# AroneyS/galah

Measured on AMD Instinct MI355X. Metric: precluster genome-pairs/sec at 10k genomes (s=1000) + sketch Gbases/s, higher is better.
Workload: dtype u64; 1 GPU; C3: 10000 synthetic genomes x 3000000 bp, clusters of 10, sub rate U(0,0.07), k=21, s=1000, min_ani=0.95; genomes=10000, genome_len=3000000, sketch_size=1000, k=21, parallelism=dp1, mode=lib

## Files before the change

### galah_amd/csrc/api.cpp

```cpp
#include <hip/hip_runtime.h>

#include <algorithm>
#include <chrono>
#include <cmath>
#include <cstdio>
#include <cstdlib>
#include <cstring>
#include <map>
#include <mutex>
#include <new>
#include <string>
#include <thread>
#include <vector>

#include "context.hpp"


namespace gg {

thread_local std::string g_thread_err;

void set_thread_error(const std::string& msg) { g_thread_err = msg; }

gg_status fail(gg_ctx* c, gg_status st, const std::string& msg) {
  if (c) c->err = msg;
  set_thread_error(msg);
  return st;
}

gg_status hip_fail(gg_ctx* c, hipError_t e, const char* what) {
  return fail(c, e == hipErrorOutOfMemory ? GG_ERR_OUT_OF_MEMORY : GG_ERR_HIP,
              std::string(what) + ": " + hipGetErrorString(e));
}

hipError_t scratch(gg_ctx* c, const char* key, size_t bytes, void** out) {
  auto& e = c->scratch[key];
  if (e.second < bytes) {
// ... 733 lines not shown
  a.overflow = b.flags + 2;
  {
    const char* e = getenv("GALAHGPU_INDEX_COST");
    const double k = !weigh_cost ? 0.0 : e && *e ? atof(e) : 0.0;
    const uint64_t n_new = n - n_old;
    const uint64_t npairs = n_old ? n_new * n_old + n_new * (n_new - 1) / 2 : pairs_in_tiles(n, tb, te);
    const double lim = k * (double)c->s * (double)npairs;
    a.cost = b.cost;
    a.cost_limit = k > 0 && lim < 1.8e19 ? (unsigned long long)lim : ~0ull;
  }
  uint64_t* d_count0;
  GG_HIP(c, scratch_t(c, "idx_count0", 1, &d_count0));
  GG_HIP(c, hipMemcpyAsync(d_count0, d_count, sizeof(uint64_t), hipMemcpyDeviceToDevice, st));
  auto launch_pairs = [&](bool guarded) -> gg_status {
    a.build_flags = guarded ? b.flags : nullptr;
    a.ents16 = b.bucket && index_ents16(n);
    GG_HIP(c, timed_launch(c, GG_KERNEL_PAIRS, work, st, [&] { return launch_index_pairs(a, r1 - r0, st); }));
    return GG_OK;
  };
  uint64_t info[2] = {0, 0};
  uint32_t kept = 0;
  uint32_t flags[4] = {0, 0, 0, 0};
  bool built = false, paired = false;
  if (b.bucket && !b.bloom) {
    const uint32_t nbb = index_bucket_bound(total);
    const char* se = getenv("GALAHGPU_INDEX_SPLIT");
    const bool split = !(se && *se == '0');
    if (split) {
      GG_HIP(c, scratch_t(c, "idx_split_cnt", (size_t)256 * n + 1, &b.split_cnt));
      GG_HIP(c, scratch_t(c, "idx_split_off", (size_t)256 * n + 1, &b.split_off));
      GG_HIP(c, scratch_t(c, "idx_split_hist", (size_t)256 * 16 * 256, &b.split_hist));
    }
    b.sort_tmp_bytes = split ? index_split_tmp_bytes(n) : index_bucket_sort_tmp_bytes(total);
    GG_HIP(c, scratch(c, "idx_sort_tmp", b.sort_tmp_bytes, &b.sort_tmp));
    GG_HIP(c, scratch_t(c, "idx_bstart", split ? (size_t)65537 : (size_t)nbb + 1, &b.bstart));
    GG_HIP(c, timed_launch(c, GG_KERNEL_PAIRS_INDEX, total, st, [&] { return index_fill(b, st); }));
    GG_HIP(c, timed_launch(c, GG_KERNEL_PAIRS_INDEX, 0, st, [&] { return index_build_buckets(b, total, nbb, st); }));
    gg_status ps = launch_pairs(true);
    if (ps != GG_OK) return ps;
    uint64_t* h_if;
    GG_HIP(c, host_scratch_t(c, "idx_info", 5, &h_if));
    GG_HIP(c, hipMemcpyAsync(h_if, b.info, 5 * sizeof(uint64_t), hipMemcpyDeviceToHost, st));
    GG_HIP(c, hipStreamSynchronize(st));
    memcpy(info, h_if, sizeof info);
    memcpy(flags, h_if + 2, sizeof flags);
    built = paired = flags[3] == 0;
    if (built && !flags[0] && h_if[4] > a.cost_limit) {
      *costly = true;
      return GG_OK;
    }
  } else {
    uint32_t nbuckets = 0;
    GG_HIP(c, timed_launch(c, GG_KERNEL_PAIRS_INDEX, total, st, [&] { return index_fill(b, st); }));
    GG_HIP(c, hipMemcpyAsync(info, b.info, sizeof info, hipMemcpyDeviceToHost, st));
    if (b.bloom) GG_HIP(c, hipMemcpyAsync(&kept, b.flags + 1, sizeof kept, hipMemcpyDeviceToHost, st));
    if (b.bucket)
      GG_HIP(c, hipMemcpyAsync(&nbuckets, b.bbase + kIndexCoarse, sizeof nbuckets, hipMemcpyDeviceToHost, st));
    GG_HIP(c, hipStreamSynchronize(st));
    if (b.bucket) {
      b.sort_tmp_bytes = index_bucket_sort_tmp_bytes(kept);
      GG_HIP(c, scratch(c, "idx_sort_tmp", b.sort_tmp_bytes, &b.sort_tmp));
      GG_HIP(c, scratch_t(c, "idx_bstart", (size_t)nbuckets + 1, &b.bstart));
      GG_HIP(c, timed_launch(c, GG_KERNEL_PAIRS_INDEX, 0, st,
                             [&] { return index_build_buckets(b, kept, nbuckets, st); }));
      GG_HIP(c, hipMemcpyAsync(flags, b.flags, sizeof flags, hipMemcpyDeviceToHost, st));
      GG_HIP(c, hipStreamSynchronize(st));
      built = flags[3] == 0;
    }
  }
// ... 23 lines not shown
    }
    a.big_map = h_if[5] > kBigMapRun;
  } else if (!paired && !flags[0]) {
    uint64_t cost[2] = {0, 0};
    GG_HIP(c, hipMemcpyAsync(cost, b.info + 4, sizeof cost, hipMemcpyDeviceToHost, st));
    GG_HIP(c, hipStreamSynchronize(st));
    if (cost[0] > a.cost_limit) {
      *costly = true;
      return GG_OK;
    }
    a.big_map = cost[1] > kBigMapRun;
  }
  if (flags[0]) return GG_OK;
  if (!paired) {
    gg_status ps = launch_pairs(false);
    if (ps != GG_OK) return ps;
    GG_HIP(c, hipMemcpyAsync(&flags[2], b.flags + 2, sizeof(uint32_t), hipMemcpyDeviceToHost, st));
    GG_HIP(c, hipStreamSynchronize(st));
  }
  *used = true;
  if (flags[2]) {
    GG_HIP(c, hipMemcpyAsync(d_count, d_count0, sizeof(uint64_t), hipMemcpyDeviceToDevice, st));
    *used = false;
  }
  return GG_OK;
}

}

gg_status pairs_tables(gg_ctx* c, float min_ani, uint32_t** d_cmin, uint32_t** d_sufmin, hipStream_t st) {
  return ensure_cmin(c, min_ani, d_cmin, d_sufmin, st);
}

gg_status sorted_pairs_device(gg_ctx* c, const gg_pair* d_pairs, uint64_t cnt, uint32_t n, gg_pair** d_sorted,
                              hipStream_t st) {
  uint64_t* d_kv;
  void* d_tmp;
  const size_t tmp_bytes = pair_sort_tmp_bytes(cnt, n);
  GG_HIP(c, scratch_t(c, "pair_sort_kv", 5 * std::max<uint64_t>(cnt, 1), &d_kv));
  GG_HIP(c, scratch(c, "pair_sort_tmp", std::max<size_t>(tmp_bytes, 16), &d_tmp));
  uint32_t* d_idx = (uint32_t*)(d_kv + 2 * cnt);
  *d_sorted = (gg_pair*)(d_kv + 3 * cnt);
  if (cnt == 0) return GG_OK;
  GG_HIP(c, sort_pairs_device(d_pairs, cnt, n, d_kv, d_kv + cnt, d_idx, d_idx + cnt, *d_sorted, d_tmp, tmp_bytes, st));
  return GG_OK;
}
// ... 66 lines not shown
                           hipMemcpyHostToDevice, st));
  if (kern == 1) {
    PairsTableLaunch b;
    b.sketches = d_sk;
    b.lens = d_lens;
    b.n = n;
    b.stride = c->s;
    b.segs = d_segs;
    b.n_segs = (uint32_t)c->seg_host.size();
    b.cmin = d_cmin;
    b.tmax = 2 * c->s;
    b.out = d_out;
    b.out_cap = cap;
    b.count = (unsigned long long*)d_count;
    GG_HIP(c, timed_launch(c, GG_KERNEL_PAIRS, work, st, [&] { return launch_pairs_table(b, st); }));
    return GG_OK;
  }
#endif
  return GG_OK;
}

gg_status pairs_range_to_host(gg_ctx* c, const uint64_t* d_sk, const uint32_t* d_lens, uint32_t n,
                              uint64_t tb, uint64_t te, float min_ani, std::vector<gg_pair>& res,
                              hipStream_t st, uint32_t n_old) {
  if (n < 2 || tb >= te) return GG_OK;
  uint64_t *d_count, *h_count;
  GG_HIP(c, scratch_t(c, "pair_count", 1, &d_count));
  GG_HIP(c, host_scratch_t(c, "pair_count", 1, &h_count));
  uint64_t cap = std::max<uint64_t>(1 << 20, (uint64_t)n * 16);
  const uint64_t all = (uint64_t)n * (n > 0 ? n - 1 : 0) / 2;
  cap = std::min<uint64_t>(cap, std::max<uint64_t>(all, 1));
  for (int attempt = 0; attempt < 2; ++attempt) {
    gg_pair* d_out;
    GG_HIP(c, scratch_t(c, "pair_out", cap, &d_out));
    GG_HIP(c, hipMemsetAsync(d_count, 0, sizeof(uint64_t), st));
    gg_status ps = pairs_core(c, d_sk, d_lens, n, tb, te, min_ani, d_out, cap, d_count, st, n_old);
    if (ps != GG_OK) return ps;
    GG_HIP(c, hipMemcpyAsync(h_count, d_count, sizeof(uint64_t), hipMemcpyDeviceToHost, st));
    GG_HIP(c, hipStreamSynchronize(st));
    const uint64_t cnt = *h_count;
    if (cnt <= cap) {
      const size_t at = res.size();
      res.resize(at + cnt);
      if (cnt < kDeviceSortPairs || cnt >= (1ull << 31)) {
        if (cnt) {
          GG_HIP(c, hipMemcpyAsync(res.data() + at, d_out, cnt * sizeof(gg_pair), hipMemcpyDeviceToHost, st));
          GG_HIP(c, hipStreamSynchronize(st));
          std::sort(res.begin() + at, res.end(), [](const gg_pair& x, const gg_pair& y) {
            return x.i != y.i ? x.i < y.i : x.j < y.j;
          });
        }
        return GG_OK;
      }
      uint64_t* d_kv;
      void* d_tmp;
      const size_t tmp_bytes = pair_sort_tmp_bytes(cnt, n);
      GG_HIP(c, scratch_t(c, "pair_sort_kv", 5 * cnt, &d_kv));
      GG_HIP(c, scratch(c, "pair_sort_tmp", std::max<size_t>(tmp_bytes, 16), &d_tmp));
      uint32_t* d_idx = (uint32_t*)(d_kv + 2 * cnt);
      gg_pair* d_sorted = (gg_pair*)(d_kv + 3 * cnt);
      GG_HIP(c, sort_pairs_device(d_out, cnt, n, d_kv, d_kv + cnt, d_idx, d_idx + cnt, d_sorted, d_tmp, tmp_bytes,
                                  st));
      constexpr uint64_t kPairStage = 1ull << 20;
      gg_pair* h_sorted;
      GG_HIP(c, host_scratch_t(c, "pair_sorted", std::min(cnt, kPairStage), &h_sorted));
      for (uint64_t x = 0; x < cnt; x += kPairStage) {
        const uint64_t m = std::min(kPairStage, cnt - x);
        GG_HIP(c, hipMemcpyAsync(h_sorted, d_sorted + x, m * sizeof(gg_pair), hipMemcpyDeviceToHost, st));
        GG_HIP(c, hipStreamSynchronize(st));
        memcpy(res.data() + at + x, h_sorted, m * sizeof(gg_pair));
      }
      return GG_OK;
    }
    cap = cnt;
  }
  return fail(c, GG_ERR_INTERNAL, "pair output sizing failed");
}

double ani_f64(uint32_t common, uint32_t total, int k) {
  const double jaccard = (double)common / (double)total;
  double d = -1.0 * std::log((2.0 * jaccard) / (1.0 + jaccard)) / (double)k;
  d = rust_max(rust_min(d, 1.0), 0.0);
  return 1.0 - d;
}

std::vector<uint32_t> build_cmin(uint32_t s, int k, float min_ani) {
  const uint32_t tmax = 2 * s;
  const double thr = (double)min_ani;
  std::vector<uint32_t> cmin(tmax + 1, 0xFFFFFFFFu);
  for (uint32_t t = 0; t <= tmax; ++t) {
    const uint32_t cmax = std::min(t, s);
    if (!(ani_f64(cmax, t, k) >= thr)) continue;
    uint32_t lo = 0, hi = cmax;
// ... 514 lines not shown
```

### galah_amd/csrc/context.hpp

```cpp
#pragma once

#include <hip/hip_runtime.h>

#include <condition_variable>
#include <cstdlib>
#include <cstring>
#include <functional>
#include <map>
#include <memory>
#include <mutex>
#include <string>
#include <thread>
#include <vector>

#include "gg_internal.hpp"

class MemberPool {
 public:
  explicit MemberPool(size_t n) {
    for (size_t i = 1; i < n; ++i) th_.emplace_back([this, i] { loop(i); });
  }
  ~MemberPool() {
    {
      std::lock_guard<std::mutex> lk(mu_);
// ... 82 lines not shown
  std::unique_ptr<MemberPool> pool;
  std::vector<hipStream_t> peer_streams;
  uint64_t pair_paths[GG_PATH_COUNT] = {};
  int pairs_path = GG_PAIRS_PATH_DEFAULT;
  uint64_t pairs_paths_taken[3] = {};
  uint64_t index_costly = 0;
  uint64_t fallbacks[GG_FALLBACK_COUNT] = {};
  uint64_t inflate_dev_batches = 0;
  uint64_t gz_member_plans = 0, gz_full_plans = 0;
  uint64_t gz_scratch_bytes = 0;
  uint64_t cluster_calls = 0, cluster_rounds = 0;
  uint64_t precluster_calls = 0, precluster_jumps = 0;
  uint64_t scratch_regrows = 0;
  double scratch_regrow_ms = 0;
  double scratch_hint = 1.0;
  std::vector<uint8_t> peer_direct;
  std::vector<hipEvent_t> rep_start, rep_done;
  std::vector<char> rep_live;
  hipEvent_t rows_ready = nullptr;
  hipStream_t copy_stream = nullptr;
  hipEvent_t copy_done = nullptr;
  int host_threads = 0;
  double phase_ms[GG_PHASE_COUNT] = {0};
};

namespace gg {

inline gg_ctx* primary(gg_ctx* c) { return c && !c->devs.empty() ? c->devs[0] : c; }

gg_status fail(gg_ctx* c, gg_status st, const std::string& msg);
gg_status hip_fail(gg_ctx* c, hipError_t e, const char* what);

#define GG_HIP(ctx, expr)                                        \
  do {                                                           \
    hipError_t _e = (expr);                                      \
    if (_e != hipSuccess) return ::gg::hip_fail((ctx), _e, #expr); \
  } while (0)

hipError_t scratch(gg_ctx* c, const char* key, size_t bytes, void** out);
template <typename T>
hipError_t scratch_t(gg_ctx* c, const char* key, size_t count, T** out) {
  void* p = nullptr;
  hipError_t e = scratch(c, key, count * sizeof(T), &p);
  *out = (T*)p;
  return e;
}
hipError_t pinned(gg_ctx* c, size_t bytes, void** out);
hipError_t host_scratch(gg_ctx* c, const char* key, size_t bytes, void** out);
template <typename T>
hipError_t host_scratch_t(gg_ctx* c, const char* key, size_t count, T** out) {
  void* p = nullptr;
  hipError_t e = host_scratch(c, key, count * sizeof(T), &p);
  *out = static_cast<T*>(p);
  return e;
}

gg_status check_runs(gg_ctx* c, const gg_run* runs, uint64_t n_runs, uint32_t n_genomes, uint64_t n_words);
gg_status sketch_core(gg_ctx* c, const uint32_t* d_words, uint64_t n_words, const gg_run* runs,
                      uint64_t n_runs, uint32_t n_genomes, uint64_t* d_out, uint32_t* d_lens,
                      const uint32_t* d_row_of, hipStream_t st);
gg_status pairs_core(gg_ctx* c, const uint64_t* d_sk, const uint32_t* d_lens, uint32_t n,
                     uint64_t tb, uint64_t te, float min_ani, gg_pair* d_out, uint64_t cap,
                     uint64_t* d_count, hipStream_t st, uint32_t n_old = 0);
constexpr uint64_t kDeviceSortPairs = 4096;
gg_status pairs_range_to_host(gg_ctx* c, const uint64_t* d_sk, const uint32_t* d_lens, uint32_t n,
                              uint64_t tb, uint64_t te, float min_ani, std::vector<gg_pair>& res,
                              hipStream_t st, uint32_t n_old = 0);

gg_status cluster_device(gg_ctx* c, uint32_t n, const gg_pair* d_pairs, const float* d_ani, uint64_t n_pairs, float T,
                         uint32_t* d_rep_of, hipStream_t st);
gg_status preclusters_device(gg_ctx* c, uint32_t n, const gg_pair* d_pairs, uint64_t n_pairs, uint32_t* d_members,
                             uint32_t* d_offsets, uint32_t* n_sets, gg_local_pair* d_local, uint64_t* d_pair_offsets,
                             hipStream_t st);
gg_status ani_f32_device(gg_ctx* c, const gg_pair* d_pairs, uint64_t n_pairs, float* d_ani, double* d_ani_f64,
                         uint64_t* n_rechecked, hipStream_t st);
struct AniFlagged;
using AniProducer = std::function<hipError_t(double E, AniFlagged* list, uint64_t cap, unsigned long long* count)>;
gg_status ani_flagged_passes(gg_ctx* c, const char* who, uint64_t n_items, const AniProducer& produce, float* d_ani,
                             double* d_ani_f64, uint32_t mirror_m, uint64_t* n_flagged, hipStream_t st);
gg_status ani_matrix_device(gg_ctx* c, const uint64_t* d_sk, const uint32_t* d_lens, uint32_t n, const uint32_t* d_rows,
                            uint32_t m, uint32_t* d_common, uint32_t* d_total, float* d_ani, gg_matrix_summary* sum,
                            hipStream_t st);
gg_status ani_matrix_groups_device(gg_ctx* c, const uint64_t* d_sk, const uint32_t* d_lens, uint32_t n,
                                   const uint32_t* d_members, const uint32_t* offsets, uint32_t n_groups,
                                   uint32_t* d_common, uint32_t* d_total, float* d_ani, gg_matrix_summary* sum,
                                   hipStream_t st);
struct MatrixPrep {
  const uint32_t *pos_row, *pos_len, *piece, *piece_cnt;
  uint32_t m;
  uint64_t n_entries, n_columns, column_entries;
// ... 85 lines not shown
```

### galah_amd/csrc/gg_internal.hpp

```cpp
#pragma once

#include <hip/hip_runtime.h>

#include <cstdint>
#include <memory>
#include <string>
#include <vector>

#include "../../include/galahgpu.h"

namespace gg {

constexpr uint64_t kEmpty = ~0ull;

enum SketchStatus : uint32_t {
  kSketchOk = 0,
  kSketchRetryLarger = 1,
  kSketchRetrySmaller = 2,
  kSketchRetrySet = 3,
};

constexpr uint32_t kFlagOverflow = 1u;
constexpr uint32_t kFlagSawMax = 2u;
constexpr uint32_t kFlagSetMode = 4u;
// ... 317 lines not shown
  unsigned long long* count;
  uint32_t max_split_log2;
  uint32_t* overflow;
  const uint32_t* build_flags = nullptr;
  bool ents16 = false;
  const unsigned long long* cost = nullptr;
  unsigned long long cost_limit = ~0ull;
  bool big_map = false;
  bool border = false;
};
hipError_t index_fill(const IndexBuild& b, hipStream_t st);
hipError_t index_build(const IndexBuild& b, uint64_t total, uint32_t sh, uint32_t end_bit, hipStream_t st);
hipError_t index_build_buckets(const IndexBuild& b, uint64_t total, uint32_t nb_bound, hipStream_t st);
uint32_t index_bucket_bound(uint64_t entries);
size_t index_cost_bytes();
size_t index_sort_tmp_bytes(uint64_t total, uint32_t end_bit);
size_t index_bucket_sort_tmp_bytes(uint64_t total);
size_t index_split_tmp_bytes(uint32_t n);
constexpr uint32_t kIndexCoarse = 4096;
hipError_t launch_index_pairs(const IndexLaunch& a, uint32_t n_rows, hipStream_t st);
bool index_ents16(uint32_t n);
uint32_t pair_key_bits(uint32_t n);
size_t pair_sort_tmp_bytes(uint64_t cnt, uint32_t n);
hipError_t sort_pairs_device(const gg_pair* d_pairs, uint64_t cnt, uint32_t n, uint64_t* keys, uint64_t* keys_out,
                             uint32_t* idx, uint32_t* idx_out, gg_pair* sorted, void* tmp, size_t tmp_bytes,
                             hipStream_t st);

hipError_t launch_synth(uint32_t first_genome, uint32_t n_genomes, uint32_t genome_len,
                        uint32_t cluster_size, float max_sub_rate,
                        uint64_t seed, uint32_t* words, hipStream_t st);

hipError_t launch_synth_mixed(uint32_t first_genome, uint32_t n_genomes, const uint64_t* d_woff,
                              uint64_t max_words, uint32_t cluster_size, float max_sub_rate, uint64_t seed,
                              uint32_t* words, hipStream_t st);

struct FileStamp {
  uint64_t size = 0;
  int64_t mtime_ns = 0;
  bool ok = false;
};
bool file_stamp(const char* path, FileStamp* out);

int ingest_threads(int n_threads);
class PackStream {
 public:
  PackStream(const char* const* paths, uint32_t n, int k, int n_threads, uint64_t budget_bytes,
             bool stamp_files = false, bool raw = false, bool stats = false);
  ~PackStream();
  PackStream(const PackStream&) = delete;
// ... 32 lines not shown
```

### galah_amd/csrc/multi.cpp

```cpp
#include <algorithm>
#include <chrono>
#include <future>
#include <cstdio>
#include <cstring>
#include <mutex>
#include <new>
#include <thread>

#include "context.hpp"

namespace gg {
namespace {

using Clock = std::chrono::steady_clock;
double ms_since(Clock::time_point t0) {
  return std::chrono::duration<double, std::milli>(Clock::now() - t0).count();
}

std::vector<gg_ctx*> members(gg_ctx* c) { return c->devs.empty() ? std::vector<gg_ctx*>{c} : c->devs; }

template <class F>
gg_status on_members(gg_ctx* c, const std::vector<gg_ctx*>& ms, F&& f) {
  std::vector<gg_status> st(ms.size(), GG_OK);
  const std::function<void(size_t)> run = [&](size_t i) {
// ... 79 lines not shown
  }
  for (size_t o = 0; o < M; ++o)
    if (m->rep_live[o]) {
      GG_HIP(m, hipEventRecord(m->rep_done[o], m->peer_streams[o]));
      GG_HIP(m, hipStreamWaitEvent(m->stream, m->rep_done[o], 0));
    }
  return GG_OK;
}

double replicate_ms(gg_ctx* m) {
  double worst = 0.0;
  for (size_t o = 0; o < m->rep_live.size(); ++o) {
    if (!m->rep_live[o]) continue;
    float ms = 0.f;
    if (hipEventElapsedTime(&ms, m->rep_start[o], m->rep_done[o]) == hipSuccess) worst = std::max(worst, (double)ms);
  }
  return worst;
}

bool pair_ij_less(const gg_pair& x, const gg_pair& y) { return x.i != y.i ? x.i < y.i : x.j < y.j; }

gg_status gather_pairs_merge(gg_ctx* c, const std::vector<gg_ctx*>& ms, const std::vector<Rows>& rows,
                             const std::vector<RowSpan>& spans, uint32_t n, float min_ani,
                             std::vector<gg_pair>& res) {
  const size_t M = ms.size();
  auto t0 = Clock::now();
  std::vector<std::vector<gg_pair>> part(M);
  const uint64_t nb = (n + GG_PAIR_TILE - 1) / GG_PAIR_TILE;
  const bool by_rows = M > 1 && min_ani > 0.0f && !(min_ani != min_ani);
  auto row_tile = [&](uint64_t I) { return I * nb - I * (I - 1) / 2; };
  gg_status st = on_members(c, ms, [&](size_t i, gg_ctx* m) {
    uint64_t tb = 0, te = 0;
    if (by_rows) {
      tb = row_tile(nb * i / M);
      te = row_tile(nb * (i + 1) / M);
    } else {
      gg_pair_partition(n, (uint32_t)M, (uint32_t)i, &tb, &te);
    }
    if (M > 1 && !spans.empty()) {
      const gg_status r = replicate(m, i, ms, rows, spans, c->peer_direct);
      if (r != GG_OK) return r;
    }
    return pairs_range_to_host(m, rows[i].sk, rows[i].len, n, tb, te, min_ani, part[i], m->stream);
  });
  if (st != GG_OK) return st;
  c->phase_ms[GG_PHASE_PAIRS] = ms_since(t0);
  double rep = 0.0;
  if (M > 1 && !spans.empty())
    for (gg_ctx* m : ms) rep = std::max(rep, replicate_ms(m));
  c->phase_ms[GG_PHASE_REPLICATE] = rep;
  t0 = Clock::now();
  res.clear();
  size_t total = 0;
  bool ordered = true;
  const gg_pair* last = nullptr;
  for (const auto& p : part) {
    if (p.empty()) continue;
    total += p.size();
    if (last && !pair_ij_less(*last, p.front())) ordered = false;
    last = &p.back();
  }
  if (ordered) {
    for (auto& p : part) {
      if (p.empty()) continue;
      if (res.empty() && p.size() == total) {
        res.swap(p);
        break;
      }
      if (res.empty()) res.reserve(total);
      res.insert(res.end(), p.begin(), p.end());
    }
  } else {
    for (auto& p : part) {
      if (res.empty()) {
        res.swap(p);
        continue;
      }
      std::vector<gg_pair> merged(res.size() + p.size());
      std::merge(res.begin(), res.end(), p.begin(), p.end(), merged.begin(), pair_ij_less);
      res.swap(merged);
    }
  }
  c->phase_ms[GG_PHASE_MERGE] = ms_since(t0);
  return GG_OK;
}

gg_status pairs_with_ani(gg_ctx* c, const std::vector<gg_pair>& res, gg_pair** pairs, float** ani,
                         uint64_t* n_out) {
  auto t0 = Clock::now();
  const size_t m = res.size();
  *pairs = copy_out(res);
  *ani = (float*)malloc(std::max<size_t>(m, 1) * sizeof(float));
  if (!*pairs || !*ani) {
    free(*pairs);
    free(*ani);
    *pairs = nullptr;
    *ani = nullptr;
    return fail(c, GG_ERR_OUT_OF_MEMORY, "out of host memory");
  }
  float* a = *ani;
  const int T = m >= (1u << 16) ? (int)std::min<size_t>(16, std::max(1, ingest_threads(c->host_threads))) : 1;
  std::vector<std::thread> th;
  auto work = [&](int t) {
    for (size_t i = m * t / T; i < m * (t + 1) / T; ++i) a[i] = gg_ani_f32(res[i].common, res[i].total, c->k);
  };
  for (int t = 1; t < T; ++t) th.emplace_back(work, t);
  work(0);
  for (auto& x : th) x.join();
  *n_out = m;
  c->phase_ms[GG_PHASE_MERGE] += ms_since(t0);
  return GG_OK;
}

constexpr uint32_t kBatchGenomes = 32;
constexpr uint64_t kBatchWords = 64ull << 20;
constexpr uint64_t kBatchText = 1ull << 30;
void parallel_copy(void* dst, const void* src, size_t bytes, int T) {
  constexpr size_t kPer = 8u << 20;
  T = (int)std::max<size_t>(1, std::min<size_t>((size_t)T, bytes / kPer));
  if (T <= 1) {
    if (bytes) memcpy(dst, src, bytes);
    return;
  }
// ... 723 lines not shown
                              out_stats);
}

gg_status gg_precluster_files_cached(gg_ctx* ctx, const char* const* paths, uint32_t n_paths, float min_ani,
                                     const char* cache_dir, gg_pair** pairs, float** ani, uint64_t* n_out,
                                     uint32_t* n_cached) {
  if (!ctx) return fail(nullptr, GG_ERR_INVALID_ARG, "null context");
  if (!pairs || !ani || !n_out || (n_paths && !paths))
    return fail(ctx, GG_ERR_INVALID_ARG, "gg_precluster_files: null argument");
  if (std::isnan(min_ani)) return fail(ctx, GG_ERR_INVALID_ARG, "min_ani is NaN");
  *pairs = nullptr;
  *ani = nullptr;
  *n_out = 0;
  if (n_cached) *n_cached = 0;
  for (double& x : ctx->phase_ms) x = 0.0;
  const std::vector<gg_ctx*> ms = members(ctx);
  std::vector<Rows> rows;
  std::vector<RowSpan> spans;
  std::vector<gg_pair> res;
  auto t0 = Clock::now();
  gg_status st = sketch_files_members(ctx, ms, paths, n_paths, cache_dir, rows, spans, nullptr, nullptr, n_cached);
  if (st != GG_OK) return st;
  ctx->phase_ms[GG_PHASE_SKETCH] = ms_since(t0);
  if (n_paths >= 2) {
    st = gather_pairs_merge(ctx, ms, rows, spans, n_paths, min_ani, res);
    if (st != GG_OK) return st;
  }
  return pairs_with_ani(ctx, res, pairs, ani, n_out);
}

gg_status gg_precluster_files(gg_ctx* ctx, const char* const* paths, uint32_t n_paths, float min_ani,
                              gg_pair** pairs, float** ani, uint64_t* n_out) {
  return gg_precluster_files_cached(ctx, paths, n_paths, min_ani, nullptr, pairs, ani, n_out, nullptr);
}

gg_status gg_cluster_files_resident(gg_ctx* ctx, const char* const* paths, uint32_t n_paths, float min_ani,
                                    float cluster_ani, const char* cache_dir, uint32_t* rep_of,
                                    gg_cluster_summary* summary) {
  if (!ctx) return fail(nullptr, GG_ERR_INVALID_ARG, "null context");
  if (summary) *summary = gg_cluster_summary{};
  if (n_paths && (!paths || !rep_of)) return fail(ctx, GG_ERR_INVALID_ARG, "gg_cluster_files_resident: null argument");
  if (std::isnan(min_ani) || std::isnan(cluster_ani))
    return fail(ctx, GG_ERR_INVALID_ARG, "gg_cluster_files_resident: min_ani or cluster_ani is NaN");
  const std::vector<gg_ctx*> ms = members(ctx);
  if (ms.size() > 1) {
    gg_pair* p = nullptr;
    float* a = nullptr;
    uint64_t n = 0;
    gg_status st = gg_cluster_files(ctx, paths, n_paths, min_ani, cluster_ani, cache_dir, rep_of, &p, &a, &n);
    if (st == GG_OK && summary && n_paths) {
      std::vector<uint32_t> mem(n_paths), off((size_t)n_paths + 1);
// ... 310 lines not shown
      return fail(ctx, GG_ERR_INVALID_ARG, "gg_precluster_shards: null shard buffer");
    if ((uint64_t)off[i] + shards[i].n_genomes > 0xFFFFFFFFull)
      return fail(ctx, GG_ERR_INVALID_ARG, "gg_precluster_shards: too many genomes");
    off[i + 1] = off[i] + shards[i].n_genomes;
  }
  const uint32_t n = off[M];
  std::vector<Rows> rows(M);
  std::vector<RowSpan> spans;
  for (size_t i = 0; i < M; ++i)
    if (shards[i].n_genomes) spans.push_back(RowSpan{off[i], shards[i].n_genomes, (uint32_t)i});
  auto t0 = Clock::now();
  gg_status st = on_members(ctx, ms, [&](size_t mi, gg_ctx* m) -> gg_status {
    gg_status r = member_rows(m, n, &rows[mi]);
    if (r != GG_OK) return r;
    const gg_shard& sh = shards[mi];
    if (sh.n_genomes == 0) return GG_OK;
    const gg_status ks = sketch_core(m, sh.d_words, sh.n_words, sh.runs, sh.n_runs, sh.n_genomes,
                                     rows[mi].sk + (size_t)off[mi] * m->s, rows[mi].len + off[mi], nullptr, m->stream);
    return ks != GG_OK ? ks : mark_rows_ready(m);
  });
  if (st != GG_OK) return st;
  ctx->phase_ms[GG_PHASE_SKETCH] = ms_since(t0);
  std::vector<gg_pair> res;
  if (n >= 2) {
    st = gather_pairs_merge(ctx, ms, rows, spans, n, min_ani, res);
    if (st != GG_OK) return st;
  }
  return pairs_with_ani(ctx, res, pairs, ani, n_out);
}

}
```

### galah_amd/csrc/pairs_index.hip

```cpp
#include <hipcub/hipcub.hpp>

#include <algorithm>

#include "device_util.hpp"
#include "gg_internal.hpp"

namespace gg {
namespace {

constexpr int kRowThreads = 256;
constexpr int kScanThreads = 1024;
constexpr uint32_t kXcds = 8;

struct KeyShape {
  uint32_t sh, norm;
};
__device__ __forceinline__ KeyShape key_shape(unsigned long long maxh) {
  const uint32_t bits = maxh ? 64u - (uint32_t)__builtin_clzll(maxh) : 0u;
  const uint32_t sh = bits > 32 ? bits - 32 : 0u;
  const uint32_t eb = bits - sh > 1u ? bits - sh : 1u;
  return KeyShape{sh, 32u - eb};
}

constexpr uint32_t kCoarseBits = 12;
constexpr uint32_t kBucketPad = 0xFFFFu;
constexpr uint32_t kBucketKeyBits = 16;
constexpr uint32_t kCoarse = 1u << kCoarseBits;
__device__ __forceinline__ uint32_t bucket_of(uint64_t h, KeyShape ks, const uint32_t* __restrict__ bbase) {
// ... 28 lines not shown
    sum += l;
    if (l) mx = max(mx, (unsigned long long)sk[(uint64_t)i * stride + l - 1]);
  }
  unsigned long long inc = sum;
  for (int o = 1; o < 64; o <<= 1) {
    const unsigned long long y = __shfl_up(inc, o);
    if ((tid & 63) >= (uint32_t)o) inc += y;
  }
  for (int o = 32; o > 0; o >>= 1) mx = max(mx, (unsigned long long)__shfl_xor(mx, o));
  if ((tid & 63) == 63) wsum[tid >> 6] = inc;
  if ((tid & 63) == 0) wmax[tid >> 6] = mx;
  __syncthreads();
  unsigned long long run = inc - sum;
  for (uint32_t w = 0; w < (tid >> 6); ++w) run += wsum[w];
  for (uint32_t i = b0; i < b1; ++i) {
    offs[i] = run;
    run += lens[i];
  }
  if (tid == kScanThreads - 1) {
    info[0] = run;
    unsigned long long m = 0;
    for (int w = 0; w < kScanThreads / 64; ++w) m = max(m, wmax[w]);
    info[1] = m;
  }
}

template <bool BUCKET>
__global__ __launch_bounds__(256) void index_fill_kernel(const uint64_t* __restrict__ sk,
                                                         const uint32_t* __restrict__ lens,
                                                         const uint64_t* __restrict__ offs, uint32_t n,
                                                         uint32_t stride, uint32_t kbits, uint32_t sh,
                                                         const unsigned long long* __restrict__ info,
                                                         const uint32_t* __restrict__ bbase,
                                                         uint32_t* __restrict__ keys, uint64_t* __restrict__ vals) {
  const KeyShape ks = BUCKET ? key_shape(info[1]) : KeyShape{sh, 0u};
  for (uint32_t i = blockIdx.x; i < n; i += gridDim.x) {
    const uint32_t len = lens[i];
    const uint64_t* row = sk + (uint64_t)i * stride;
    if (BUCKET) {
      const uint64_t o = (uint64_t)i * stride;
      for (uint32_t k = threadIdx.x; k < stride; k += 256) {
        ((uint16_t*)keys)[o + k] = (uint16_t)(k < len ? bucket_of(row[k], ks, bbase) : kBucketPad);
        ((uint32_t*)vals)[o + k] = (i << kbits) | k;
      }
      continue;
    }
// ... 14 lines not shown
  const uint32_t prev = __shfl_up(v, 1);
  const bool head = in && (lane == 0 || prev != v);
  const uint64_t heads = __ballot(head);
  const uint32_t n_in = (uint32_t)__popcll(__ballot(in));
  if (head) {
    const uint64_t after = (heads >> lane) >> 1;
    const uint32_t next = after ? lane + 1u + (uint32_t)__builtin_ctzll(after) : 64u;
    atomicAdd(&h[v], (min(next, n_in) - lane) * weight);
  }
}

__global__ __launch_bounds__(256) void bucket_hist_kernel(const uint64_t* __restrict__ sk,
                                                          const uint32_t* __restrict__ lens, uint32_t n,
                                                          uint32_t stride,
                                                          const unsigned long long* __restrict__ info,
                                                          uint32_t* __restrict__ hist, uint32_t may_sample) {
  __shared__ uint32_t lh[kCoarse];
  for (uint32_t x = threadIdx.x; x < kCoarse; x += 256) lh[x] = 0u;
  __syncthreads();
  const KeyShape ks = key_shape(info[1]);
  const uint32_t i0 = (uint32_t)((uint64_t)n * blockIdx.x / gridDim.x);
  const uint32_t i1 = (uint32_t)((uint64_t)n * (blockIdx.x + 1) / gridDim.x);
  auto bin = [&](uint64_t h) { return ((uint32_t)(h >> ks.sh) << ks.norm) >> (32 - kCoarseBits); };
  const bool sample = may_sample && info[0] >= (1ull << 26);
  for (uint32_t i = i0; i < i1; ++i) {
    const uint32_t len = lens[i];
    const uint64_t* row = sk + (uint64_t)i * stride;
    if (sample) {
      const uint32_t lines = (len + 15) / 16, first = i & 7;
      const uint32_t q_end = lines > first ? (lines - first + 7) / 8 * 16 : 0;
      for (uint32_t q0 = 0; q0 < q_end; q0 += 256) {
        const uint32_t q = q0 + threadIdx.x;
        const uint32_t k = (first + (q >> 4) * 8) * 16 + (q & 15);
        const bool in = q < q_end && k < len;
        const uint32_t b = in ? bin(row[k]) : ~0u;
        wave_runs_add(lh, b, in, 8);
      }
      continue;
    }
    for (uint32_t k0 = 0; k0 < len; k0 += 256) {
      const uint32_t k = k0 + threadIdx.x;
      const bool in = k < len;
      const uint32_t b = in ? bin(row[k]) : ~0u;
      wave_runs_add(lh, b, in);
    }
  }
  __syncthreads();
// ... 713 lines not shown
  const uint64_t t0 = rs, t1 = rs + (nb - I);
  const uint64_t a = max(t0, tb), b = min(t1, te);
  if (a >= b) {
    jlo = jhi = 0;
    return;
  }
  const uint64_t J0 = I + (a - rs), J1 = I + (b - rs);
  jlo = (uint32_t)max<uint64_t>(J0 * GG_PAIR_TILE, (uint64_t)i + 1);
  jhi = (uint32_t)min<uint64_t>(J1 * GG_PAIR_TILE, (uint64_t)n);
}

__device__ __forceinline__ uint32_t part_of(uint32_t j, uint32_t plog2) {
  return plog2 ? (j * 0x9E3779B1u) >> (32 - plog2) : 0u;
}

constexpr uint32_t kMemberLoads = 8;
template <bool E16, uint32_t MAPLOG2, bool BORDER = false>
__global__ __launch_bounds__(kRowThreads) void index_pairs_kernel(IndexLaunch a) {
  constexpr uint32_t kMapLog2 = MAPLOG2, kMap = 1u << kMapLog2, kMapFull = kMap * 3 / 4;
  __shared__ uint32_t mkey[kMap];
  __shared__ uint32_t mcnt[kMap];
  __shared__ uint32_t fill;
  __shared__ volatile uint32_t over;
  const uint32_t tid = threadIdx.x;
  const uint32_t per_xcd = (a.n_rows + kXcds - 1) / kXcds;
  const uint32_t ri_ = (blockIdx.x % kXcds) * per_xcd + blockIdx.x / kXcds;
  if (ri_ >= a.n_rows) return;
  const uint32_t i = a.row0 + ri_;
  if (i >= a.n) return;
  if (a.build_flags && ((a.build_flags[0] | a.build_flags[3]) || (a.cost && *a.cost > a.cost_limit))) return;
  uint32_t jlo, jhi;
  if (BORDER) jlo = 0u, jhi = i;
  else row_columns(i, a.n, a.nb, a.tile_begin, a.tile_end, jlo, jhi);
  const uint32_t la = a.lens[i];
  if (jlo >= jhi || la == 0) return;
  const uint64_t* ri = a.runinfo + (uint64_t)i * a.stride;
  const uint64_t* A = a.sketches + (uint64_t)i * a.stride;
  const uint64_t xa = A[la - 1];
  uint32_t plog2 = 0;
  for (uint32_t p = 0; p < (1u << plog2);) {
    for (uint32_t x = tid; x < kMap; x += kRowThreads) mkey[x] = 0u, mcnt[x] = 0u;
    if (tid == 0) fill = 0u, over = 0u;
    __syncthreads();
    uint64_t info_next = tid < la ? ri[tid] : 0ull;
    for (uint32_t k = tid; k < la; k += kRowThreads) {
      if (over) break;
// ... 27 lines not shown
            }
            if (probe >= kMap) {
              over = 1u;
              break;
            }
            h = (h + 1) & (kMap - 1);
          }
          if (over) stop = true;
        }
      }
      if (stop) break;
    }
    __syncthreads();
    if (over) {
      if (plog2 < a.max_split_log2) {
        ++plog2;
        p *= 2;
        __syncthreads();
        continue;
      }
      if (tid == 0) atomicOr(a.overflow, 1u);
      return;
    }
    for (uint32_t x = tid; x < kMap; x += kRowThreads) {
      const uint32_t key = mkey[x];
      if (!key) continue;
      const uint32_t j = key - 1u, common = mcnt[x];
      const uint32_t lb = a.lens[j];
      if (common < a.sufmin[min(la, lb)]) continue;
      const uint64_t* B = a.sketches + (uint64_t)j * a.stride;
      const uint64_t xb = B[lb - 1];
      const uint32_t total = xa <= xb ? la + count_le(B, lb, xa) - common : count_le(A, la, xb) + lb - common;
      if (total <= a.tmax && common >= a.cmin[total]) {
        const unsigned long long slot = atomicAdd(a.count, 1ull);
        if (slot < a.out_cap) a.out[slot] = BORDER ? gg_pair{j, i, common, total} : gg_pair{i, j, common, total};
      }
    }
    __syncthreads();
    ++p;
  }
}

}

static bool hist_sampling() {
  const char* e = getenv("GALAHGPU_INDEX_HIST_SAMPLE");
  return !(e && *e == '0');
}

hipError_t index_fill(const IndexBuild& b, hipStream_t st) {
  hipError_t e = hipMemsetAsync(b.flags, 0, 4 * sizeof(uint32_t) + index_cost_bytes(), st);
  if (e != hipSuccess) return e;
  hipLaunchKernelGGL(index_scan_kernel, dim3(1), dim3(kScanThreads), 0, st, b.sketches, b.lens, b.n, b.stride,
                     b.offs, (unsigned long long*)b.info);
  e = hipGetLastError();
  if (e != hipSuccess) return e;
  const unsigned long long* info = (const unsigned long long*)b.info;
  if (b.bucket) {
    e = hipMemsetAsync(b.hist, 0, kCoarse * sizeof(uint32_t), st);
    if (e != hipSuccess) return e;
    hipLaunchKernelGGL(bucket_hist_kernel, dim3(std::max(1u, std::min<uint32_t>(b.n, 1024))), dim3(256), 0, st,
                       b.sketches, b.lens, b.n, b.stride, info, b.hist, hist_sampling() ? 1u : 0u);
    hipLaunchKernelGGL(bucket_base_kernel, dim3(1), dim3(kBaseThreads), 0, st, b.hist, info, b.bbase);
    e = hipGetLastError();
    if (e != hipSuccess) return e;
  }
  if (!b.bloom) return hipSuccess;
  e = hipMemsetAsync(b.bloom, 0, ((size_t)1 << b.bloom_log2) / 8, st);
  if (e != hipSuccess) return e;
  if (b.r1 > b.r0)
    hipLaunchKernelGGL(bloom_build_kernel, dim3(std::min<uint32_t>(b.r1 - b.r0, 16384)), dim3(256), 0, st,
                       b.sketches, b.lens, b.r0, b.r1, b.stride, b.bloom, b.bloom_log2);
  const dim3 grid(std::max(1u, std::min<uint32_t>(b.n, 4096)));
  if (b.bucket)
    hipLaunchKernelGGL(index_fill_range_kernel<true>, grid, dim3(256), 0, st, b.sketches, b.lens, b.n, b.stride,
                       b.kbits, b.bloom, b.bloom_log2, b.r0, b.r1, info, b.bbase, b.flags + 1, b.keys_in, b.vals_in);
  else
// ... 157 lines not shown
      if (a.big_map) hipLaunchKernelGGL((index_pairs_kernel<false, 13, true>), grid, dim3(kRowThreads), 0, st, b);
      else hipLaunchKernelGGL((index_pairs_kernel<false, 11, true>), grid, dim3(kRowThreads), 0, st, b);
    }
  } else if (a.ents16) {
    if (a.big_map) hipLaunchKernelGGL((index_pairs_kernel<true, 13>), grid, dim3(kRowThreads), 0, st, b);
    else hipLaunchKernelGGL((index_pairs_kernel<true, 11>), grid, dim3(kRowThreads), 0, st, b);
  } else {
    if (a.big_map) hipLaunchKernelGGL((index_pairs_kernel<false, 13>), grid, dim3(kRowThreads), 0, st, b);
    else hipLaunchKernelGGL((index_pairs_kernel<false, 11>), grid, dim3(kRowThreads), 0, st, b);
  }
  return hipGetLastError();
}

namespace {
__global__ __launch_bounds__(256) void pair_keys_kernel(const gg_pair* __restrict__ p, uint32_t cnt, uint32_t n,
                                                        uint64_t* __restrict__ keys, uint32_t* __restrict__ idx) {
  for (uint32_t x = blockIdx.x * 256 + threadIdx.x; x < cnt; x += gridDim.x * 256) {
    const gg_pair q = p[x];
    keys[x] = (uint64_t)q.i * n + q.j;
    idx[x] = x;
  }
}

__global__ __launch_bounds__(256) void pair_gather_kernel(const gg_pair* __restrict__ p, uint32_t cnt,
                                                          const uint32_t* __restrict__ idx,
                                                          gg_pair* __restrict__ sorted) {
  for (uint32_t y = blockIdx.x * 256 + threadIdx.x; y < cnt; y += gridDim.x * 256) sorted[y] = p[idx[y]];
}
}

uint32_t pair_key_bits(uint32_t n) {
  const uint64_t mx = (uint64_t)n * n;
  uint32_t bits = 1;
  while (bits < 64 && (mx >> bits) != 0) ++bits;
  return bits;
}

size_t pair_sort_tmp_bytes(uint64_t cnt, uint32_t n) {
  size_t bytes = 0;
  (void)hipcub::DeviceRadixSort::SortPairs(nullptr, bytes, (const uint64_t*)nullptr, (uint64_t*)nullptr,
                                           (const uint32_t*)nullptr, (uint32_t*)nullptr, (int)cnt, 0,
                                           (int)pair_key_bits(n));
  return bytes;
}

hipError_t sort_pairs_device(const gg_pair* d_pairs, uint64_t cnt, uint32_t n, uint64_t* keys, uint64_t* keys_out,
                             uint32_t* idx, uint32_t* idx_out, gg_pair* sorted, void* tmp, size_t tmp_bytes,
                             hipStream_t st) {
  if (cnt == 0) return hipSuccess;
  if (cnt >= (1ull << 31)) return hipErrorInvalidValue;
  const dim3 grid((uint32_t)std::min<uint64_t>(4096, (cnt + 255) / 256));
  hipLaunchKernelGGL(pair_keys_kernel, grid, dim3(256), 0, st, d_pairs, (uint32_t)cnt, n, keys, idx);
  hipError_t e = hipGetLastError();
  if (e != hipSuccess) return e;
  e = hipcub::DeviceRadixSort::SortPairs(tmp, tmp_bytes, keys, keys_out, idx, idx_out, (int)cnt, 0,
                                         (int)pair_key_bits(n), st);
  if (e != hipSuccess) return e;
  hipLaunchKernelGGL(pair_gather_kernel, grid, dim3(256), 0, st, d_pairs, (uint32_t)cnt, idx_out, sorted);
  return hipGetLastError();
}

bool index_ents16(uint32_t n) { return n <= 65536u; }

}
```

Before: 1.100 billion genome-pairs/s.

## Aggregate pair output atomics, fuse ANI into gather, skip count readback

```diff
diff --git a/galah_amd/csrc/api.cpp b/galah_amd/csrc/api.cpp
--- a/galah_amd/csrc/api.cpp
+++ b/galah_amd/csrc/api.cpp
@@ -13,6 +13,7 @@
 #include <thread>
 #include <vector>
 
+#include "ani_core.hpp"
 #include "context.hpp"
 
 
@@ -792,6 +793,7 @@
   uint32_t kept = 0;
   uint32_t flags[4] = {0, 0, 0, 0};
   bool built = false, paired = false;
+  uint64_t count_seen = 0;
   if (b.bucket && !b.bloom) {
     const uint32_t nbb = index_bucket_bound(total);
     const char* se = getenv("GALAHGPU_INDEX_SPLIT");
@@ -809,12 +811,14 @@
     gg_status ps = launch_pairs(true);
     if (ps != GG_OK) return ps;
     uint64_t* h_if;
-    GG_HIP(c, host_scratch_t(c, "idx_info", 5, &h_if));
+    GG_HIP(c, host_scratch_t(c, "idx_info", 6, &h_if));
     GG_HIP(c, hipMemcpyAsync(h_if, b.info, 5 * sizeof(uint64_t), hipMemcpyDeviceToHost, st));
+    GG_HIP(c, hipMemcpyAsync(h_if + 5, d_count, sizeof(uint64_t), hipMemcpyDeviceToHost, st));
     GG_HIP(c, hipStreamSynchronize(st));
     memcpy(info, h_if, sizeof info);
     memcpy(flags, h_if + 2, sizeof flags);
     built = paired = flags[3] == 0;
+    count_seen = h_if[5];
     if (built && !flags[0] && h_if[4] > a.cost_limit) {
       *costly = true;
       return GG_OK;
@@ -884,6 +888,9 @@
   if (flags[2]) {
     GG_HIP(c, hipMemcpyAsync(d_count, d_count0, sizeof(uint64_t), hipMemcpyDeviceToDevice, st));
     *used = false;
+  } else if (paired) {
+    c->pair_count_seen = true;
+    c->pair_count_host = count_seen;
   }
   return GG_OK;
 }
@@ -996,7 +1003,13 @@
 
 gg_status pairs_range_to_host(gg_ctx* c, const uint64_t* d_sk, const uint32_t* d_lens, uint32_t n,
                               uint64_t tb, uint64_t te, float min_ani, std::vector<gg_pair>& res,
-                              hipStream_t st, uint32_t n_old) {
+                              hipStream_t st, uint32_t n_old, std::vector<float>* ani) {
+  auto host_ani = [&](size_t at) {
+    if (!ani) return;
+    ani->resize(res.size());
+    for (size_t p = at; p < res.size(); ++p) (*ani)[p] = gg_ani_f32(res[p].common, res[p].total, c->k);
+  };
+  if (ani && ani->size() != res.size()) return fail(c, GG_ERR_INTERNAL, "pairs_range_to_host: ani out of step");
   if (n < 2 || tb >= te) return GG_OK;
   uint64_t *d_count, *h_count;
   GG_HIP(c, scratch_t(c, "pair_count", 1, &d_count));
@@ -1008,11 +1021,14 @@
     gg_pair* d_out;
     GG_HIP(c, scratch_t(c, "pair_out", cap, &d_out));
     GG_HIP(c, hipMemsetAsync(d_count, 0, sizeof(uint64_t), st));
+    c->pair_count_seen = false;
     gg_status ps = pairs_core(c, d_sk, d_lens, n, tb, te, min_ani, d_out, cap, d_count, st, n_old);
     if (ps != GG_OK) return ps;
-    GG_HIP(c, hipMemcpyAsync(h_count, d_count, sizeof(uint64_t), hipMemcpyDeviceToHost, st));
-    GG_HIP(c, hipStreamSynchronize(st));
-    const uint64_t cnt = *h_count;
+    if (!c->pair_count_seen) {
+      GG_HIP(c, hipMemcpyAsync(h_count, d_count, sizeof(uint64_t), hipMemcpyDeviceToHost, st));
+      GG_HIP(c, hipStreamSynchronize(st));
+    }
+    const uint64_t cnt = c->pair_count_seen ? c->pair_count_host : *h_count;
     if (cnt <= cap) {
       const size_t at = res.size();
       res.resize(at + cnt);
@@ -1024,6 +1040,7 @@
             return x.i != y.i ? x.i < y.i : x.j < y.j;
           });
         }
+        host_ani(at);
         return GG_OK;
       }
       uint64_t* d_kv;
@@ -1033,16 +1050,31 @@
       GG_HIP(c, scratch(c, "pair_sort_tmp", std::max<size_t>(tmp_bytes, 16), &d_tmp));
       uint32_t* d_idx = (uint32_t*)(d_kv + 2 * cnt);
       gg_pair* d_sorted = (gg_pair*)(d_kv + 3 * cnt);
+      float* d_ani = ani ? (float*)d_idx : nullptr;
+      int margin = ani::kMarginLog2;
+      if (const char* e = getenv("GALAHGPU_TEST_ANI_MARGIN_LOG2")) margin = std::max(-1000, std::min(1000, atoi(e)));
       GG_HIP(c, sort_pairs_device(d_out, cnt, n, d_kv, d_kv + cnt, d_idx, d_idx + cnt, d_sorted, d_tmp, tmp_bytes,
-                                  st));
+                                  st, d_ani, c->k, ani::pow2(margin)));
       constexpr uint64_t kPairStage = 1ull << 20;
       gg_pair* h_sorted;
+      float* h_ani = nullptr;
       GG_HIP(c, host_scratch_t(c, "pair_sorted", std::min(cnt, kPairStage), &h_sorted));
+      if (ani) {
+        GG_HIP(c, host_scratch_t(c, "pair_sorted_ani", std::min(cnt, kPairStage), &h_ani));
+        ani->resize(at + cnt);
+      }
       for (uint64_t x = 0; x < cnt; x += kPairStage) {
         const uint64_t m = std::min(kPairStage, cnt - x);
         GG_HIP(c, hipMemcpyAsync(h_sorted, d_sorted + x, m * sizeof(gg_pair), hipMemcpyDeviceToHost, st));
+        if (ani) GG_HIP(c, hipMemcpyAsync(h_ani, d_ani + x, m * sizeof(float), hipMemcpyDeviceToHost, st));
         GG_HIP(c, hipStreamSynchronize(st));
         memcpy(res.data() + at + x, h_sorted, m * sizeof(gg_pair));
+        if (ani) {
+          float* a = ani->data() + at + x;
+          memcpy(a, h_ani, m * sizeof(float));
+          for (uint64_t q = 0; q < m; ++q)
+            if (a[q] == kAniRecheck) a[q] = gg_ani_f32(h_sorted[q].common, h_sorted[q].total, c->k);
+        }
       }
       return GG_OK;
     }
diff --git a/galah_amd/csrc/context.hpp b/galah_amd/csrc/context.hpp
--- a/galah_amd/csrc/context.hpp
+++ b/galah_amd/csrc/context.hpp
@@ -128,6 +128,8 @@
   hipEvent_t copy_done = nullptr;
   int host_threads = 0;
   double phase_ms[GG_PHASE_COUNT] = {0};
+  bool pair_count_seen = false;
+  uint64_t pair_count_host = 0;
 };
 
 namespace gg {
@@ -171,7 +173,7 @@
 constexpr uint64_t kDeviceSortPairs = 4096;
 gg_status pairs_range_to_host(gg_ctx* c, const uint64_t* d_sk, const uint32_t* d_lens, uint32_t n,
                               uint64_t tb, uint64_t te, float min_ani, std::vector<gg_pair>& res,
-                              hipStream_t st, uint32_t n_old = 0);
+                              hipStream_t st, uint32_t n_old = 0, std::vector<float>* ani = nullptr);
 
 gg_status cluster_device(gg_ctx* c, uint32_t n, const gg_pair* d_pairs, const float* d_ani, uint64_t n_pairs, float T,
                          uint32_t* d_rep_of, hipStream_t st);
diff --git a/galah_amd/csrc/gg_internal.hpp b/galah_amd/csrc/gg_internal.hpp
--- a/galah_amd/csrc/gg_internal.hpp
+++ b/galah_amd/csrc/gg_internal.hpp
@@ -363,9 +363,10 @@
 bool index_ents16(uint32_t n);
 uint32_t pair_key_bits(uint32_t n);
 size_t pair_sort_tmp_bytes(uint64_t cnt, uint32_t n);
+constexpr float kAniRecheck = -1.0f;
 hipError_t sort_pairs_device(const gg_pair* d_pairs, uint64_t cnt, uint32_t n, uint64_t* keys, uint64_t* keys_out,
                              uint32_t* idx, uint32_t* idx_out, gg_pair* sorted, void* tmp, size_t tmp_bytes,
-                             hipStream_t st);
+                             hipStream_t st, float* ani = nullptr, int k = 0, double E = 0.0);
 
 hipError_t launch_synth(uint32_t first_genome, uint32_t n_genomes, uint32_t genome_len,
                         uint32_t cluster_size, float max_sub_rate,
diff --git a/galah_amd/csrc/multi.cpp b/galah_amd/csrc/multi.cpp
--- a/galah_amd/csrc/multi.cpp
+++ b/galah_amd/csrc/multi.cpp
@@ -125,8 +125,10 @@
 
 gg_status gather_pairs_merge(gg_ctx* c, const std::vector<gg_ctx*>& ms, const std::vector<Rows>& rows,
                              const std::vector<RowSpan>& spans, uint32_t n, float min_ani,
-                             std::vector<gg_pair>& res) {
+                             std::vector<gg_pair>& res, std::vector<float>* ani = nullptr) {
   const size_t M = ms.size();
+  if (ani) ani->clear();
+  std::vector<float>* ani0 = M == 1 ? ani : nullptr;
   auto t0 = Clock::now();
   std::vector<std::vector<gg_pair>> part(M);
   const uint64_t nb = (n + GG_PAIR_TILE - 1) / GG_PAIR_TILE;
@@ -144,7 +146,7 @@
       const gg_status r = replicate(m, i, ms, rows, spans, c->peer_direct);
       if (r != GG_OK) return r;
     }
-    return pairs_range_to_host(m, rows[i].sk, rows[i].len, n, tb, te, min_ani, part[i], m->stream);
+    return pairs_range_to_host(m, rows[i].sk, rows[i].len, n, tb, te, min_ani, part[i], m->stream, 0, ani0);
   });
   if (st != GG_OK) return st;
   c->phase_ms[GG_PHASE_PAIRS] = ms_since(t0);
@@ -189,7 +191,7 @@
 }
 
 gg_status pairs_with_ani(gg_ctx* c, const std::vector<gg_pair>& res, gg_pair** pairs, float** ani,
-                         uint64_t* n_out) {
+                         uint64_t* n_out, const std::vector<float>* have = nullptr) {
   auto t0 = Clock::now();
   const size_t m = res.size();
   *pairs = copy_out(res);
@@ -202,6 +204,12 @@
     return fail(c, GG_ERR_OUT_OF_MEMORY, "out of host memory");
   }
   float* a = *ani;
+  if (have && have->size() == m && m) {
+    memcpy(a, have->data(), m * sizeof(float));
+    *n_out = m;
+    c->phase_ms[GG_PHASE_MERGE] += ms_since(t0);
+    return GG_OK;
+  }
   const int T = m >= (1u << 16) ? (int)std::min<size_t>(16, std::max(1, ingest_threads(c->host_threads))) : 1;
   std::vector<std::thread> th;
   auto work = [&](int t) {
@@ -971,11 +979,12 @@
   gg_status st = sketch_files_members(ctx, ms, paths, n_paths, cache_dir, rows, spans, nullptr, nullptr, n_cached);
   if (st != GG_OK) return st;
   ctx->phase_ms[GG_PHASE_SKETCH] = ms_since(t0);
+  std::vector<float> res_ani;
   if (n_paths >= 2) {
-    st = gather_pairs_merge(ctx, ms, rows, spans, n_paths, min_ani, res);
+    st = gather_pairs_merge(ctx, ms, rows, spans, n_paths, min_ani, res, &res_ani);
     if (st != GG_OK) return st;
   }
-  return pairs_with_ani(ctx, res, pairs, ani, n_out);
+  return pairs_with_ani(ctx, res, pairs, ani, n_out, &res_ani);
 }
 
 gg_status gg_precluster_files(gg_ctx* ctx, const char* const* paths, uint32_t n_paths, float min_ani,
@@ -1332,11 +1341,12 @@
   if (st != GG_OK) return st;
   ctx->phase_ms[GG_PHASE_SKETCH] = ms_since(t0);
   std::vector<gg_pair> res;
+  std::vector<float> res_ani;
   if (n >= 2) {
-    st = gather_pairs_merge(ctx, ms, rows, spans, n, min_ani, res);
+    st = gather_pairs_merge(ctx, ms, rows, spans, n, min_ani, res, &res_ani);
     if (st != GG_OK) return st;
   }
-  return pairs_with_ani(ctx, res, pairs, ani, n_out);
-}
-
-}
+  return pairs_with_ani(ctx, res, pairs, ani, n_out, &res_ani);
+}
+
+}
diff --git a/galah_amd/csrc/pairs_index.hip b/galah_amd/csrc/pairs_index.hip
--- a/galah_amd/csrc/pairs_index.hip
+++ b/galah_amd/csrc/pairs_index.hip
@@ -2,8 +2,11 @@
 
 #include <algorithm>
 
+#include "ani_core.hpp"
+#include "ani_flag.hpp"
 #include "device_util.hpp"
 #include "gg_internal.hpp"
+#include "pairs_out_core.hpp"
 
 namespace gg {
 namespace {
@@ -78,6 +81,28 @@
     unsigned long long m = 0;
     for (int w = 0; w < kScanThreads / 64; ++w) m = max(m, wmax[w]);
     info[1] = m;
+  }
+}
+
+__global__ __launch_bounds__(256) void index_info_kernel(const uint64_t* __restrict__ sk,
+                                                         const uint32_t* __restrict__ lens, uint32_t n,
+                                                         uint32_t stride, unsigned long long* __restrict__ info) {
+  __shared__ unsigned long long wsum[256 / 64], wmax[256 / 64];
+  const uint32_t tid = threadIdx.x, i = blockIdx.x * 256 + tid;
+  const uint32_t l = i < n ? lens[i] : 0u;
+  unsigned long long sum = l, mx = l ? (unsigned long long)sk[(uint64_t)i * stride + l - 1] : 0ull;
+  for (int o = 32; o > 0; o >>= 1) {
+    sum += __shfl_xor(sum, o);
+    mx = max(mx, (unsigned long long)__shfl_xor(mx, o));
+  }
+  if ((tid & 63) == 0) wsum[tid >> 6] = sum, wmax[tid >> 6] = mx;
+  __syncthreads();
+  if (tid == 0) {
+    for (uint32_t w = 1; w < 256 / 64; ++w) sum += wsum[w], mx = max(mx, wmax[w]);
+    if (sum) {
+      atomicAdd(&info[0], sum);
+      atomicMax(&info[1], mx);
+    }
   }
 }
 
@@ -138,7 +163,7 @@
   const uint32_t i0 = (uint32_t)((uint64_t)n * blockIdx.x / gridDim.x);
   const uint32_t i1 = (uint32_t)((uint64_t)n * (blockIdx.x + 1) / gridDim.x);
   auto bin = [&](uint64_t h) { return ((uint32_t)(h >> ks.sh) << ks.norm) >> (32 - kCoarseBits); };
-  const bool sample = may_sample && info[0] >= (1ull << 26);
+  const bool sample = may_sample && info[0] >= (1ull << 22);
   for (uint32_t i = i0; i < i1; ++i) {
     const uint32_t len = lens[i];
     const uint64_t* row = sk + (uint64_t)i * stride;
@@ -898,6 +923,10 @@
   __shared__ uint32_t mcnt[kMap];
   __shared__ uint32_t fill;
   __shared__ volatile uint32_t over;
+  constexpr uint32_t kSweep = 8;
+  static_assert(kMap % (kRowThreads * kSweep) == 0, "output sweeps cover the map");
+  __shared__ uint32_t wout[kRowThreads / 64];
+  __shared__ unsigned long long obase;
   const uint32_t tid = threadIdx.x;
   const uint32_t per_xcd = (a.n_rows + kXcds - 1) / kXcds;
   const uint32_t ri_ = (blockIdx.x % kXcds) * per_xcd + blockIdx.x / kXcds;
@@ -971,21 +1000,50 @@
       if (tid == 0) atomicOr(a.overflow, 1u);
       return;
     }
-    for (uint32_t x = tid; x < kMap; x += kRowThreads) {
-      const uint32_t key = mkey[x];
-      if (!key) continue;
-      const uint32_t j = key - 1u, common = mcnt[x];
-      const uint32_t lb = a.lens[j];
-      if (common < a.sufmin[min(la, lb)]) continue;
-      const uint64_t* B = a.sketches + (uint64_t)j * a.stride;
-      const uint64_t xb = B[lb - 1];
-      const uint32_t total = xa <= xb ? la + count_le(B, lb, xa) - common : count_le(A, la, xb) + lb - common;
-      if (total <= a.tmax && common >= a.cmin[total]) {
-        const unsigned long long slot = atomicAdd(a.count, 1ull);
-        if (slot < a.out_cap) a.out[slot] = BORDER ? gg_pair{j, i, common, total} : gg_pair{i, j, common, total};
-      }
-    }
-    __syncthreads();
+    for (uint32_t x0 = 0; x0 < kMap; x0 += kRowThreads * kSweep) {
+      uint32_t pj[kSweep], pc[kSweep], pt[kSweep], np = 0;
+#pragma unroll
+      for (uint32_t u = 0; u < kSweep; ++u) {
+        const uint32_t x = x0 + u * kRowThreads + tid;
+        pj[u] = ~0u;
+        pc[u] = pt[u] = 0u;
+        const uint32_t key = mkey[x];
+        if (!key) continue;
+        const uint32_t j = key - 1u, common = mcnt[x];
+        const uint32_t lb = a.lens[j];
+        if (common < a.sufmin[min(la, lb)]) continue;
+        const uint64_t* B = a.sketches + (uint64_t)j * a.stride;
+        const uint64_t xb = B[lb - 1];
+        const uint32_t total = xa <= xb ? la + count_le(B, lb, xa) - common : count_le(A, la, xb) + lb - common;
+        if (total <= a.tmax && common >= a.cmin[total]) {
+          pj[u] = j;
+          pc[u] = common;
+          pt[u] = total;
+          ++np;
+        }
+      }
+      uint32_t inc = np;
+      for (int o = 1; o < 64; o <<= 1) {
+        const uint32_t y = __shfl_up(inc, o);
+        if ((tid & 63) >= (uint32_t)o) inc += y;
+      }
+      if ((tid & 63) == 63) wout[tid >> 6] = inc;
+      __syncthreads();
+      if (tid == 0) {
+        const uint32_t tot = pairs_out::block_total(wout, kRowThreads / 64);
+        obase = tot ? atomicAdd(a.count, (unsigned long long)tot) : 0ull;
+      }
+      __syncthreads();
+      unsigned long long slot = pairs_out::first_slot(obase, wout, tid >> 6, inc, np);
+#pragma unroll
+      for (uint32_t u = 0; u < kSweep; ++u) {
+        if (pj[u] == ~0u) continue;
+        if (slot < a.out_cap)
+          a.out[slot] = BORDER ? gg_pair{pj[u], i, pc[u], pt[u]} : gg_pair{i, pj[u], pc[u], pt[u]};
+        ++slot;
+      }
+      __syncthreads();
+    }
     ++p;
   }
 }
@@ -998,10 +1056,18 @@
 }
 
 hipError_t index_fill(const IndexBuild& b, hipStream_t st) {
-  hipError_t e = hipMemsetAsync(b.flags, 0, 4 * sizeof(uint32_t) + index_cost_bytes(), st);
-  if (e != hipSuccess) return e;
-  hipLaunchKernelGGL(index_scan_kernel, dim3(1), dim3(kScanThreads), 0, st, b.sketches, b.lens, b.n, b.stride,
-                     b.offs, (unsigned long long*)b.info);
+  hipError_t e;
+  if (b.bucket && (const void*)(b.info + 2) == (const void*)b.flags) {
+    e = hipMemsetAsync(b.info, 0, 2 * sizeof(uint64_t) + 4 * sizeof(uint32_t) + index_cost_bytes(), st);
+    if (e != hipSuccess) return e;
+    hipLaunchKernelGGL(index_info_kernel, dim3((b.n + 255) / 256), dim3(256), 0, st, b.sketches, b.lens, b.n,
+                       b.stride, (unsigned long long*)b.info);
+  } else {
+    e = hipMemsetAsync(b.flags, 0, 4 * sizeof(uint32_t) + index_cost_bytes(), st);
+    if (e != hipSuccess) return e;
+    hipLaunchKernelGGL(index_scan_kernel, dim3(1), dim3(kScanThreads), 0, st, b.sketches, b.lens, b.n, b.stride,
+                       b.offs, (unsigned long long*)b.info);
+  }
   e = hipGetLastError();
   if (e != hipSuccess) return e;
   const unsigned long long* info = (const unsigned long long*)b.info;
@@ -1205,10 +1271,19 @@
   }
 }
 
+template <bool ANI>
 __global__ __launch_bounds__(256) void pair_gather_kernel(const gg_pair* __restrict__ p, uint32_t cnt,
                                                           const uint32_t* __restrict__ idx,
-                                                          gg_pair* __restrict__ sorted) {
-  for (uint32_t y = blockIdx.x * 256 + threadIdx.x; y < cnt; y += gridDim.x * 256) sorted[y] = p[idx[y]];
+                                                          gg_pair* __restrict__ sorted, float* __restrict__ ani, int k,
+                                                          double E) {
+  for (uint32_t y = blockIdx.x * 256 + threadIdx.x; y < cnt; y += gridDim.x * 256) {
+    const gg_pair q = p[idx[y]];
+    sorted[y] = q;
+    if (ANI) {
+      const ani::Value r = ani::value(q.common, q.total, k, E, DeviceLog{});
+      ani[y] = r.flagged ? kAniRecheck : r.f;
+    }
+  }
 }
 }
 
@@ -1229,7 +1304,7 @@
 
 hipError_t sort_pairs_device(const gg_pair* d_pairs, uint64_t cnt, uint32_t n, uint64_t* keys, uint64_t* keys_out,
                              uint32_t* idx, uint32_t* idx_out, gg_pair* sorted, void* tmp, size_t tmp_bytes,
-                             hipStream_t st) {
+                             hipStream_t st, float* ani, int k, double E) {
   if (cnt == 0) return hipSuccess;
   if (cnt >= (1ull << 31)) return hipErrorInvalidValue;
   const dim3 grid((uint32_t)std::min<uint64_t>(4096, (cnt + 255) / 256));
@@ -1239,7 +1314,12 @@
   e = hipcub::DeviceRadixSort::SortPairs(tmp, tmp_bytes, keys, keys_out, idx, idx_out, (int)cnt, 0,
                                          (int)pair_key_bits(n), st);
   if (e != hipSuccess) return e;
-  hipLaunchKernelGGL(pair_gather_kernel, grid, dim3(256), 0, st, d_pairs, (uint32_t)cnt, idx_out, sorted);
+  if (ani)
+    hipLaunchKernelGGL(pair_gather_kernel<true>, grid, dim3(256), 0, st, d_pairs, (uint32_t)cnt, idx_out, sorted, ani,
+                       k, E);
+  else
+    hipLaunchKernelGGL(pair_gather_kernel<false>, grid, dim3(256), 0, st, d_pairs, (uint32_t)cnt, idx_out, sorted,
+                       nullptr, 0, 0.0);
   return hipGetLastError();
 }
 
diff --git a/galah_amd/csrc/pairs_out_core.hpp b/galah_amd/csrc/pairs_out_core.hpp
--- /dev/null
+++ b/galah_amd/csrc/pairs_out_core.hpp
@@ -0,0 +1,28 @@
+#pragma once
+
+#include <cstdint>
+
+#if defined(__HIPCC__) || defined(__CUDACC__)
+#define GG_OUT_HD __host__ __device__
+#else
+#define GG_OUT_HD
+#endif
+
+namespace gg {
+namespace pairs_out {
+
+GG_OUT_HD inline uint32_t block_total(const uint32_t* wave_totals, uint32_t waves) {
+  uint32_t t = 0;
+  for (uint32_t w = 0; w < waves; ++w) t += wave_totals[w];
+  return t;
+}
+
+GG_OUT_HD inline unsigned long long first_slot(unsigned long long base, const uint32_t* wave_totals, uint32_t wave,
+                                               uint32_t inclusive, uint32_t own) {
+  unsigned long long s = base + (inclusive - own);
+  for (uint32_t w = 0; w < wave; ++w) s += wave_totals[w];
+  return s;
+}
+
+}
+}
```

Result: no change. 1.104 billion genome-pairs/s, median of 6 (+0.4%).
